# ambicuity/Distributed-LLM-Training-and-Inference-System

Measured on AMD Instinct MI355X. Metric: tokens/sec (node) GPT-7B train, higher is better.
Workload: dtype bf16; 1 GPU; model=gpt-7b, global_batch=16, seq_len=2048, parallelism=dp1, micro_batch=16, grad_accum=1, activation_checkpoint=none, layout=planner

## Files before the change

llmctl/ops/csrc/flash_attn_bwd.hip:

```cpp
#include <cstdlib>
#include <map>
#include <mutex>

#include "attn_common.h"

namespace llmctl {
using namespace attn;
namespace {

constexpr float LOG2E = 1.4426950408889634f;
constexpr int KV_KB = 128;
constexpr int KV_QT = 64;
#ifndef LLMCTL_DKV_NBUF
#define LLMCTL_DKV_NBUF 2
#endif
constexpr int KV_NBUF = LLMCTL_DKV_NBUF;
static_assert(KV_NBUF >= 2 && KV_NBUF <= 4, "dK/dV ring depth 2-4");
constexpr int DQ_QB = 128;
constexpr int DQ_KB = 64;

struct BwdArgs {
  const unsigned short *q, *k, *v, *dout;
  const float* lse;
  const float* delta;
// ... 509 lines not shown
  const unsigned short* qc = qh + (long)q_start * a.q_ss;
  const unsigned short* dc = dh + (long)q_start * a.do_ss;
  const long q_step = (long)KV_QT * a.q_ss, d_step = (long)KV_QT * a.do_ss;
  auto issue = [&](auto slot_c) __attribute__((always_inline)) {
    constexpr int SLC = decltype(slot_c)::value;
    const int nr = min(KV_QT, a.S - iq0);
    i32x4_t rq = buf_rsrc(qc, (unsigned)(((nr - 1) * a.q_ss + HD) * 2));
    i32x4_t rd = buf_rsrc(dc, (unsigned)(((nr - 1) * a.do_ss + HD) * 2));
    i32x4_t rr = (DOC && wave == 2) ? buf_rsrc(a.doc + (long)b * a.S + iq0, (unsigned)(nr * 4))
                                    : buf_rsrc(rh + iq0, (unsigned)(nr * 4));
    asm volatile("s_nop 4" : "+s"(rq), "+s"(rd), "+s"(rr));
    const unsigned slot = lds0 + (unsigned)(SLC * BUF_B);
#pragma unroll
    for (int i = 0; i < NP; ++i) {
      buf_dma16(rq, vq[i], slot + (i * 4 + wave) * 1024);
      buf_dma16(rd, vd[i], slot + TILE_B + (i * 4 + wave) * 1024);
    }
    buf_dma4(rr, rc_off, slot + 2 * TILE_B + wave * RC_B);
    iq0 += KV_QT;
    qc += q_step;
    dc += d_step;
    if (iq0 >= q_end) {
      iq0 = q_start;
      qh += a.q_sh;
      dh += a.do_sh;
      rh += a.S;
      qc = qh + (long)q_start * a.q_ss;
      dc = dh + (long)q_start * a.do_ss;
    }
  };

  const float c = a.scale_log2;
  auto apply_mask = [&](f32x16& s, int h, int q0, const int* doc_s) __attribute__((always_inline)) {
#pragma unroll
    for (int gq = 0; gq < 4; ++gq) {
      const int row0 = 32 * h + 8 * gq + 4 * hh;
      int sv[4] = {0, 0, 0, 0};
      if constexpr (DOC) {
        const int4 s4 = *reinterpret_cast<const int4*>(doc_s + row0);
        sv[0] = s4.x; sv[1] = s4.y; sv[2] = s4.z; sv[3] = s4.w;
      }
#pragma unroll
      for (int j = 0; j < 4; ++j) {
        const int qq = q0 + row0 + j;
        bool ok = qq < a.S && my_key < a.S;
        if constexpr (CAUSAL) ok = ok && my_key <= qq;
        if constexpr (DOC) ok = ok && my_key >= sv[j];
        s[4 * gq + j] = ok ? s[4 * gq + j] : -INFINITY;
      }
    }
  };

  if (ntiles > 0) issue(std::integral_constant<int, 0>{});
  bf16x8_t kf[NKS], vf[NKS];
  {
    const int kc = min(my_key, a.S - 1);
    const unsigned short* Kp = a.k + b * a.k_sb + hk * a.k_sh + (long)kc * a.k_ss + 8 * hh;
    const unsigned short* Vp = a.v + b * a.v_sb + hk * a.v_sh + (long)kc * a.v_ss + 8 * hh;
#pragma unroll
    for (int ks = 0; ks < NKS; ++ks) {
      asm volatile("global_load_dwordx4 %0, %1, off" : "=a"(kf[ks]) : "v"(Kp + 16 * ks) : "memory");
      asm volatile("global_load_dwordx4 %0, %1, off" : "=a"(vf[ks]) : "v"(Vp + 16 * ks) : "memory");
    }
  }
  vm_wait_n<0>();
  __builtin_amdgcn_s_barrier();
  stamp(2);
  if (ntiles > 1) issue(std::integral_constant<int, 1>{});
  int qi = 0;
  auto tile = [&](auto slot_c, int t) __attribute__((always_inline)) {
    constexpr int SL = decltype(slot_c)::value;
    const int q0 = q_start + qi * KV_QT;
    if (++qi == nq) qi = 0;
    const bool live = !(CAUSAL && wkey0 > q0 + KV_QT - 1);
    const unsigned char* Qs = smem + SL * BUF_B;
    const unsigned char* Ds = Qs + TILE_B;
    const float* lse_s = reinterpret_cast<const float*>(Ds + TILE_B);
    const float* del_s = lse_s + KV_QT;
    const int* doc_s = reinterpret_cast<const int*>(del_s + KV_QT);
    if (!live) return;
    f32x16 s0 = *reinterpret_cast<const f32x16*>(lse_s + 16 * hh);
    f32x16 p0 = *reinterpret_cast<const f32x16*>(del_s + 16 * hh);
    bf16x8_t qa[NKS], da[NKS];
#pragma unroll
    for (int ks = 0; ks < NKS; ++ks) {
      qa[ks] = lds_read_b128(Qs, tr_off<HD>(r, 2 * ks + hh));
      da[ks] = lds_read_b128(Ds, tr_off<HD>(r, 2 * ks + hh));
    }
    const bool need_mask = DOC || (CAUSAL && wkey0 + 31 > q0) || (q0 + KV_QT > a.S) || (wkey0 + 31 >= a.S);
#pragma unroll
    for (int ks = 0; ks < NKS; ++ks) {
      mfma_v(s0, qa[ks], kf[ks]);
      mfma_v(p0, da[ks], vf[ks]);
    }
    f32x16 s1 = *reinterpret_cast<const f32x16*>(lse_s + 32 + 16 * hh);
    f32x16 p1 = *reinterpret_cast<const f32x16*>(del_s + 32 + 16 * hh);
#pragma unroll
    for (int ks = 0; ks < NKS; ++ks) {
      qa[ks] = lds_read_b128(Qs, tr_off<HD>(32 + r, 2 * ks + hh));
      da[ks] = lds_read_b128(Ds, tr_off<HD>(32 + r, 2 * ks + hh));
    }
    if (need_mask) apply_mask(s0, 0, q0, doc_s);
    unsigned pw0[8], dw0[8];
    bf16x8_t td[2][NDB], tq[2][NDB];
#pragma unroll
    for (int ks = 0; ks < NKS; ++ks) {
      x_step(s1, p1, qa[ks], kf[ks], da[ks], vf[ks], s0[2 * ks], s0[2 * ks + 1], p0[2 * ks], p0[2 * ks + 1], c, pw0[ks],
             dw0[ks]);
      const int st = ks >> 2, d = ks & 3;
      td[st][d] = tr_frag<HD>(Ds, 16 * st, d * 32, lane);
      tq[st][d] = tr_frag<HD>(Qs, 16 * st, d * 32, lane);
    }
    if (need_mask) apply_mask(s1, 1, q0, doc_s);
    unsigned pw1[8], dw1[8];
    bf16x8_t cd[2][NDB], cq[2][NDB];
#pragma unroll
    for (int st = 0; st < 2; ++st) {
      const bf16x8_t pb = words8(pw0[4 * st], pw0[4 * st + 1], pw0[4 * st + 2], pw0[4 * st + 3]);
      const bf16x8_t sb = words8(dw0[4 * st], dw0[4 * st + 1], dw0[4 * st + 2], dw0[4 * st + 3]);
#pragma unroll
      for (int d = 0; d < NDB; ++d) {
        const int i = 4 * st + d;
        y_step(dv[d], dk[d], td[st][d], tq[st][d], pb, sb, s1[2 * i], s1[2 * i + 1], p1[2 * i], p1[2 * i + 1], c,
               pw1[i], dw1[i]);
        cd[st][d] = tr_frag<HD>(Ds, 32 + 16 * st, d * 32, lane);
        cq[st][d] = tr_frag<HD>(Qs, 32 + 16 * st, d * 32, lane);
      }
    }
#pragma unroll
    for (int st = 0; st < 2; ++st) {
      const bf16x8_t pb = words8(pw1[4 * st], pw1[4 * st + 1], pw1[4 * st + 2], pw1[4 * st + 3]);
      const bf16x8_t sb = words8(dw1[4 * st], dw1[4 * st + 1], dw1[4 * st + 2], dw1[4 * st + 3]);
#pragma unroll
      for (int d = 0; d < NDB; ++d) z_step(dv[d], dk[d], cd[st][d], cq[st][d], pb, sb);
    }
  };
  auto advance = [&](auto slot_c, int t) __attribute__((always_inline)) {
    constexpr int SL = decltype(slot_c)::value;
    asm volatile("s_waitcnt lgkmcnt(0)" ::: "memory");
    vm_wait_n<0>();
    __builtin_amdgcn_s_barrier();
    if (t + 2 < ntiles) issue(std::integral_constant<int, SL>{});
  };
  for (int t = 0; t < ntiles; t += 2) {
    tile(std::integral_constant<int, 0>{}, t);
    advance(std::integral_constant<int, 0>{}, t);
    if (t + 1 < ntiles) {
      tile(std::integral_constant<int, 1>{}, t + 1);
      advance(std::integral_constant<int, 1>{}, t + 1);
    }
  }
  stamp(3);
#pragma unroll
  for (int d = 0; d < NDB; ++d) asm volatile("s_nop 7\n\ts_nop 7" : "+a"(dk[d]), "+a"(dv[d]));
  if (my_key < a.S) {
    const long tok = (long)b * a.S + my_key;
    unsigned short* dkp = a.dk + tok * a.dk_st + (long)hk * HD;
    unsigned short* dvp = a.dv + tok * a.dv_st + (long)hk * HD;
    const float *cr = nullptr, *sr = nullptr;
    if (a.cos_t != nullptr) {
      const long p = a.rope_pos ? (long)a.rope_pos[tok] : tok % a.rope_S;
      cr = a.cos_t + p * (HD / 2);
      sr = a.sin_t + p * (HD / 2);
    }
    store_row<HD>(dkp, dk, a.scale, hh, cr, sr);
    store_row<HD>(dvp, dv, 1.f, hh, nullptr, nullptr);
  }
  if constexpr (STAMP) {
    asm volatile("s_waitcnt vmcnt(0)" ::: "memory");
    __syncthreads();
    stamp(4);
    if (tid == 0) a.stamps[blockIdx.x * 8 + 5] = (unsigned long long)ntiles;
  }
}

template <bool STAMP>
__global__ __launch_bounds__(256, 1) void fa_bwd_dkv_persist_kernel(BwdArgs a, int* __restrict__ wq) {
  constexpr int HD = 128;
  constexpr int NKS = HD / 16;
  constexpr int NDB = HD / 32;
  constexpr int ROWB = HD * 2;
  constexpr int TILE_B = KV_QT * ROWB;
  constexpr int NP = TILE_B / 1024 / 4;
  constexpr int RC_B = KV_QT * 4;
  constexpr int BUF_B = 2 * TILE_B + 4 * RC_B;
  __shared__ __attribute__((aligned(1024))) unsigned char smem[2 * BUF_B + 64];
  int* item_w = reinterpret_cast<int*>(smem + 2 * BUF_B);

  const int tid = threadIdx.x;
  const int lane = tid & 63;
  const int wave = __builtin_amdgcn_readfirstlane(tid >> 6);
  const int r = lane & 31, hh = lane >> 5;
  const int nkb = a.S / KV_KB;
  const int BH = a.B * a.Hkv;
  const bool per_xcd = BH % 8 == 0;
  const int xq = per_xcd ? (int)(blockIdx.x & 7) : 0;
  const int n_items = (per_xcd ? BH / 8 : BH) * nkb;
  const int bh_base = per_xcd ? xq * (BH / 8) : 0;
  const int group = a.Hq / a.Hkv;
  auto pop = [&]() __attribute__((always_inline)) -> int {
    const int j = __hip_atomic_fetch_add(wq + xq, 1, __ATOMIC_RELAXED, __HIP_MEMORY_SCOPE_AGENT);
    return j < n_items ? j : -1;
  };
  if (tid == 0) {
    const int i0 = pop();
    item_w[1] = i0;
    item_w[2] = i0 >= 0 ? pop() : -1;
  }
  __syncthreads();
  int cur = __builtin_amdgcn_readfirstlane(item_w[1]);
  int nxt = __builtin_amdgcn_readfirstlane(item_w[2]);
  if (cur < 0) return;

  const unsigned lds0 = lds_addr(smem);
  unsigned vq[NP], vd[NP];
#pragma unroll
  for (int i = 0; i < NP; ++i) {
    const int byte = (i * 4 + wave) * 1024 + lane * 16;
    const int row = byte / ROWB;
    const int lch = ((byte % ROWB) >> 4) ^ swz_tr<HD>(row);
    vq[i] = (unsigned)((row * a.q_ss + lch * 8) * 2);
    vd[i] = (unsigned)((row * a.do_ss + lch * 8) * 2);
  }
  const float* rc_src = a.rck_w + (wave == 1 ? a.rc_n : 0);
  const unsigned rc_off =
      (unsigned)((32 * (lane >> 5) + 8 * ((lane >> 2) & 3) + 4 * ((lane >> 4) & 1) + (lane & 3)) * 4);

  int iss = cur, iq0 = 0, iq_start = 0, ig = 0;
  const unsigned short *qh = nullptr, *dh = nullptr;
  const float* rh = nullptr;
  bool look_pending = false;
  int n_switch = 0;
  int pend0 = -1, pend1 = -1, npend = 0;
  auto iss_begin = [&](int item) __attribute__((always_inline)) {
    const int bh = bh_base + item / nkb, kb = item % nkb;
    const int bb = bh / a.Hkv, hkk = bh % a.Hkv;
    iq_start = kb * KV_KB;
    iq0 = iq_start;
    ig = 0;
    qh = a.q + bb * a.q_sb + (long)(hkk * group) * a.q_sh;
    dh = a.dout + bb * a.do_sb + (long)(hkk * group) * a.do_sh;
    rh = rc_src + ((long)bb * a.Hq + hkk * group) * a.S;
  };
  iss_begin(cur);
  auto issue = [&](auto slot_c) __attribute__((always_inline)) {
    constexpr int SLC = decltype(slot_c)::value;
    i32x4_t rq = buf_rsrc(qh + (long)iq0 * a.q_ss, (unsigned)(((KV_QT - 1) * a.q_ss + HD) * 2));
    i32x4_t rd = buf_rsrc(dh + (long)iq0 * a.do_ss, (unsigned)(((KV_QT - 1) * a.do_ss + HD) * 2));
    i32x4_t rr = buf_rsrc(rh + iq0, (unsigned)(KV_QT * 4));
    asm volatile("s_nop 4" : "+s"(rq), "+s"(rd), "+s"(rr));
    const unsigned slot = lds0 + (unsigned)(SLC * BUF_B);
#pragma unroll
    for (int i = 0; i < NP; ++i) {
      buf_dma16(rq, vq[i], slot + (i * 4 + wave) * 1024);
      buf_dma16(rd, vd[i], slot + TILE_B + (i * 4 + wave) * 1024);
    }
    buf_dma4(rr, rc_off, slot + 2 * TILE_B + wave * RC_B);
    iq0 += KV_QT;
    if (iq0 >= a.S) {
      if (++ig < group) {
        iq0 = iq_start;
        qh += a.q_sh;
        dh += a.do_sh;
        rh += a.S;
      } else {
        iss = nxt;
        if (iss >= 0) {
          iss_begin(iss);
          if (tid == 0) item_w[3 + (n_switch & 1)] = pop();
          look_pending = true;
          ++n_switch;
        }
        if (npend == 0) pend0 = iss;
        else pend1 = iss;
        ++npend;
      }
    }
  };

  bf16x8_t kf[NKS], vf[NKS];
  auto load_kv = [&](int item) __attribute__((always_inline)) {
    const int bh = bh_base + item / nkb, kb = item % nkb;
    const int bb = bh / a.Hkv, hkk = bh % a.Hkv;
    const int key = kb * KV_KB + wave * 32 + r;
    const unsigned short* Kp = a.k + bb * a.k_sb + hkk * a.k_sh + (long)key * a.k_ss + 8 * hh;
    const unsigned short* Vp = a.v + bb * a.v_sb + hkk * a.v_sh + (long)key * a.v_ss + 8 * hh;
#pragma unroll
    for (int ks = 0; ks < NKS; ++ks) {
      asm volatile("global_load_dwordx4 %0, %1, off" : "+a"(kf[ks]) : "v"(Kp + 16 * ks) : "memory");
      asm volatile("global_load_dwordx4 %0, %1, off" : "+a"(vf[ks]) : "v"(Vp + 16 * ks) : "memory");
    }
  };

  issue(std::integral_constant<int, 0>{});
  load_kv(cur);
  asm volatile("s_waitcnt vmcnt(0)"
               : "+a"(kf[0]), "+a"(kf[1]), "+a"(kf[2]), "+a"(kf[3]), "+a"(kf[4]), "+a"(kf[5]), "+a"(kf[6]),
                 "+a"(kf[7]), "+a"(vf[0]), "+a"(vf[1]), "+a"(vf[2]), "+a"(vf[3]), "+a"(vf[4]), "+a"(vf[5]),
                 "+a"(vf[6]), "+a"(vf[7])
               :
               : "memory");
  __builtin_amdgcn_s_barrier();
  issue(std::integral_constant<int, 1>{});
  f32x16 dk[NDB], dv[NDB];
#pragma unroll
  for (int d = 0; d < NDB; ++d) {
    const bf16x8_t z = {};
    asm volatile("s_nop 2\n\tv_mfma_f32_32x32x16_bf16 %0, %1, %1, 0" : "=a"(dk[d]) : "v"(z));
    asm volatile("v_mfma_f32_32x32x16_bf16 %0, %1, %1, 0" : "=a"(dv[d]) : "v"(z));
  }
  const float c = a.scale_log2;

  int n_done = 0;
  auto stamp = [&](int k) __attribute__((always_inline)) {
    if constexpr (STAMP) {
      if (tid == 0 && n_done < 64)
        a.stamps[(blockIdx.x * 64 + n_done) * 4 + k] = k == 3 ? (unsigned long long)cur : __builtin_amdgcn_s_memrealtime();
    }
  };
  for (;;) {
    stamp(0);
    stamp(3);
    const int bh = bh_base + cur / nkb, kb = cur % nkb;
    const int b = bh / a.Hkv, hk = bh % a.Hkv;
    const int k0 = kb * KV_KB;
    const int wkey0 = k0 + wave * 32;
    const int my_key = wkey0 + r;
    const int ntiles = group * ((a.S - k0) / KV_QT);
    int q0 = k0;
    auto apply_mask = [&](f32x16& s, int h) __attribute__((always_inline)) {
#pragma unroll
      for (int gq = 0; gq < 4; ++gq) {
        const int row0 = q0 + 32 * h + 8 * gq + 4 * hh;
#pragma unroll
        for (int j = 0; j < 4; ++j) s[4 * gq + j] = my_key <= row0 + j ? s[4 * gq + j] : -INFINITY;
      }
    };
    auto tile = [&](auto slot_c) __attribute__((always_inline)) {
      constexpr int SL = decltype(slot_c)::value;
      const bool live = !(wkey0 > q0 + KV_QT - 1);
      if (!live) return;
      const unsigned char* Qs = smem + SL * BUF_B;
      const unsigned char* Ds = Qs + TILE_B;
      const float* lse_s = reinterpret_cast<const float*>(Ds + TILE_B);
      const float* del_s = lse_s + KV_QT;
      const bool need_mask = wkey0 + 31 > q0;
      f32x16 s0 = *reinterpret_cast<const f32x16*>(lse_s + 16 * hh);
      f32x16 p0 = *reinterpret_cast<const f32x16*>(del_s + 16 * hh);
      bf16x8_t qa[NKS], da[NKS];
#pragma unroll
      for (int ks = 0; ks < NKS; ++ks) {
        qa[ks] = lds_read_b128(Qs, tr_off<HD>(r, 2 * ks + hh));
        da[ks] = lds_read_b128(Ds, tr_off<HD>(r, 2 * ks + hh));
      }
      f32x16 s1 = *reinterpret_cast<const f32x16*>(lse_s + 32 + 16 * hh);
      f32x16 p1 = *reinterpret_cast<const f32x16*>(del_s + 32 + 16 * hh);
      bf16x8_t qb[NKS], db[NKS];
#pragma unroll
      for (int ks = 0; ks < NKS; ++ks) {
        mfma_v(s0, qa[ks], kf[ks]);
        qb[ks] = lds_read_b128(Qs, tr_off<HD>(32 + r, 2 * ks + hh));
        mfma_v(p0, da[ks], vf[ks]);
        db[ks] = lds_read_b128(Ds, tr_off<HD>(32 + r, 2 * ks + hh));
      }
      if (need_mask) apply_mask(s0, 0);
      unsigned pw0[8], dw0[8];
      bf16x8_t td[2][NDB], tq[2][NDB];
#pragma unroll
      for (int ks = 0; ks < NKS; ++ks) {
        x_step(s1, p1, qb[ks], kf[ks], db[ks], vf[ks], s0[2 * ks], s0[2 * ks + 1], p0[2 * ks], p0[2 * ks + 1], c,
               pw0[ks], dw0[ks]);
        const int st = ks >> 2, d = ks & 3;
        td[st][d] = tr_frag<HD>(Ds, 16 * st, d * 32, lane);
        tq[st][d] = tr_frag<HD>(Qs, 16 * st, d * 32, lane);
      }
      if (need_mask) apply_mask(s1, 1);
      unsigned pw1[8], dw1[8];
      bf16x8_t cd[2][NDB], cq[2][NDB];
#pragma unroll
      for (int st = 0; st < 2; ++st) {
        const bf16x8_t pb = words8(pw0[4 * st], pw0[4 * st + 1], pw0[4 * st + 2], pw0[4 * st + 3]);
        const bf16x8_t sb = words8(dw0[4 * st], dw0[4 * st + 1], dw0[4 * st + 2], dw0[4 * st + 3]);
#pragma unroll
        for (int d = 0; d < NDB; ++d) {
          const int i = 4 * st + d;
          y_step(dv[d], dk[d], td[st][d], tq[st][d], pb, sb, s1[2 * i], s1[2 * i + 1], p1[2 * i], p1[2 * i + 1], c,
                 pw1[i], dw1[i]);
          cd[st][d] = tr_frag<HD>(Ds, 32 + 16 * st, d * 32, lane);
          cq[st][d] = tr_frag<HD>(Qs, 32 + 16 * st, d * 32, lane);
        }
      }
#pragma unroll
      for (int st = 0; st < 2; ++st) {
        const bf16x8_t pb = words8(pw1[4 * st], pw1[4 * st + 1], pw1[4 * st + 2], pw1[4 * st + 3]);
        const bf16x8_t sb = words8(dw1[4 * st], dw1[4 * st + 1], dw1[4 * st + 2], dw1[4 * st + 3]);
#pragma unroll
        for (int d = 0; d < NDB; ++d) z_step(dv[d], dk[d], cd[st][d], cq[st][d], pb, sb);
      }
    };
    auto advance = [&](auto slot_c) __attribute__((always_inline)) {
      constexpr int SL = decltype(slot_c)::value;
      asm volatile("s_waitcnt lgkmcnt(0)" ::: "memory");
      vm_wait_n<0>();
      __builtin_amdgcn_s_barrier();
      if (look_pending) {
        nxt = __builtin_amdgcn_readfirstlane(item_w[3 + ((n_switch - 1) & 1)]);
        look_pending = false;
      }
      if (iss >= 0) issue(std::integral_constant<int, SL>{});
      q0 += KV_QT;
      if (q0 >= a.S) q0 = k0;
    };
    for (int t = 0; t < ntiles; t += 2) {
      tile(std::integral_constant<int, 0>{});
      advance(std::integral_constant<int, 0>{});
      tile(std::integral_constant<int, 1>{});
      advance(std::integral_constant<int, 1>{});
    }
    stamp(1);
    {
      const long tok = (long)b * a.S + my_key;
      unsigned short* dkp = a.dk + tok * a.dk_st + (long)hk * HD;
      unsigned short* dvp = a.dv + tok * a.dv_st + (long)hk * HD;
      const bool rope = a.cos_t != nullptr;
      f32x4 cs[NDB / 2][4], sn[NDB / 2][4];
      if (rope) {
        const long p = a.rope_pos ? (long)a.rope_pos[tok] : tok % a.rope_S;
        const float* cr = a.cos_t + p * (HD / 2);
        const float* sr = a.sin_t + p * (HD / 2);
#pragma unroll
        for (int d = 0; d < NDB / 2; ++d)
#pragma unroll
          for (int g = 0; g < 4; ++g) {
            const int col = d * 32 + 8 * g + 4 * hh;
            cs[d][g] = *reinterpret_cast<const f32x4*>(cr + col);
            sn[d][g] = *reinterpret_cast<const f32x4*>(sr + col);
          }
      }
#pragma unroll
      for (int d = 0; d < NDB; ++d) asm volatile("s_nop 7\n\ts_nop 7" : "+a"(dk[d]), "+a"(dv[d]));
      auto st8 = [&](unsigned short* p, const float* x, float mul) __attribute__((always_inline)) {
        s2_t w;
        w[0] = (unsigned)f2bf(x[0] * mul) | ((unsigned)f2bf(x[1] * mul) << 16);
        w[1] = (unsigned)f2bf(x[2] * mul) | ((unsigned)f2bf(x[3] * mul) << 16);
        asm volatile("global_store_dwordx2 %0, %1, off" ::"v"(p), "v"(w) : "memory");
      };
#pragma unroll
      for (int d = 0; d < NDB / 2; ++d) {
        const f32x16 x1 = acc_copy(dk[d]), x2 = acc_copy(dk[d + NDB / 2]);
        acc_zero(dk[d]);
        acc_zero(dk[d + NDB / 2]);
#pragma unroll
        for (int g = 0; g < 4; ++g) {
          const int col = d * 32 + 8 * g + 4 * hh;
          float lo[4], hi[4];
#pragma unroll
          for (int j = 0; j < 4; ++j) {
            const float c1 = rope ? cs[d][g][j] : 1.f, s1 = rope ? sn[d][g][j] : 0.f;
            lo[j] = x1[4 * g + j] * c1 + x2[4 * g + j] * s1;
            hi[j] = x2[4 * g + j] * c1 - x1[4 * g + j] * s1;
          }
          st8(dkp + col, lo, a.scale);
          st8(dkp + col + HD / 2, hi, a.scale);
        }
      }
#pragma unroll
      for (int d = 0; d < NDB; ++d) {
        const f32x16 x = acc_copy(dv[d]);
        acc_zero(dv[d]);
#pragma unroll
        for (int g = 0; g < 4; ++g) {
          float y[4];
#pragma unroll
          for (int j = 0; j < 4; ++j) y[j] = x[4 * g + j];
          st8(dvp + d * 32 + 8 * g + 4 * hh, y, 1.f);
        }
      }
      load_kv(pend0 >= 0 ? pend0 : cur);
      asm volatile("s_waitcnt vmcnt(0)"
                   : "+a"(kf[0]), "+a"(kf[1]), "+a"(kf[2]), "+a"(kf[3]), "+a"(kf[4]), "+a"(kf[5]), "+a"(kf[6]),
                     "+a"(kf[7]), "+a"(vf[0]), "+a"(vf[1]), "+a"(vf[2]), "+a"(vf[3]), "+a"(vf[4]), "+a"(vf[5]),
                     "+a"(vf[6]), "+a"(vf[7])
                   :
                   : "memory");
    }
    stamp(2);
    ++n_done;
    if (pend0 < 0) break;
    cur = pend0;
    pend0 = pend1;
    pend1 = -1;
    --npend;
  }
}

template <int HD, bool CAUSAL, bool DOC>
__global__ __launch_bounds__(256, 2) void fa_bwd_dq_kernel(BwdArgs a) {
  constexpr int NKS = HD / 16;
  constexpr int NDB = HD / 32;
  constexpr int ROWB = HD * 2;
  constexpr int TILE = DQ_KB * ROWB;
  constexpr int PPW = TILE / 1024 / 4;
  constexpr int SLOT = 2 * TILE;
  __shared__ __attribute__((aligned(1024))) unsigned char smem[2 * SLOT];

  const int tid = threadIdx.x;
  const int lane = tid & 63;
  const int wave = __builtin_amdgcn_readfirstlane(tid >> 6);
  const int r = lane & 31, hh = lane >> 5;
  const int nqb = (a.S + DQ_QB - 1) / DQ_QB;
  const int BH = a.B * a.Hq;
  int bh, qi;
  if (BH % 8) {
    bh = blockIdx.x % BH;
    qi = blockIdx.x / BH;
  } else {
    const int x = blockIdx.x & 7, j = blockIdx.x >> 3;
    bh = x * (BH >> 3) + j / nqb;
    qi = j % nqb;
  }
  const int qblk = nqb - 1 - qi;
  const int b = bh / a.Hq, hq = bh % a.Hq;
  const int hk = hq / (a.Hq / a.Hkv);
  const int q_row0 = qblk * DQ_QB + wave * 32;
  const int my_q = q_row0 + r;
  const int qc = min(my_q, a.S - 1);

  const unsigned short* Kp = a.k + b * a.k_sb + hk * a.k_sh;
  const unsigned short* Vp = a.v + b * a.v_sb + hk * a.v_sh;

#pragma unroll
  for (int i = 0; i < 2 * SLOT / 4096; ++i)
    *reinterpret_cast<uint4*>(smem + i * 4096 + tid * 16) = make_uint4(0, 0, 0, 0);

  bf16x8_t qf[NKS], df[NKS];
  {
    const unsigned short* Qp = a.q + b * a.q_sb + hq * a.q_sh + (long)qc * a.q_ss + 8 * hh;
    const unsigned short* Dp = a.dout + b * a.do_sb + hq * a.do_sh + (long)qc * a.do_ss + 8 * hh;
#pragma unroll
    for (int ks = 0; ks < NKS; ++ks) {
      qf[ks] = __builtin_bit_cast(bf16x8_t, gload16(Qp + 16 * ks));
      df[ks] = __builtin_bit_cast(bf16x8_t, gload16(Dp + 16 * ks));
    }
  }
  const long rc = ((long)b * a.Hq + hq) * a.S + qc;
  const float nlse2 = -a.lse[rc] * LOG2E;
  float dlt;
  if (a.o != nullptr) {
    const unsigned short* Op = a.o + b * a.o_sb + hq * a.o_sh + (long)qc * a.o_ss + 8 * hh;
    float acc = 0.f;
#pragma unroll
    for (int ks = 0; ks < NKS; ++ks) {
      const bf16x8_t of = __builtin_bit_cast(bf16x8_t, gload16(Op + 16 * ks));
#pragma unroll
      for (int j = 0; j < 8; ++j) acc += (float)of[j] * (float)df[ks][j];
    }
    dlt = xor32_add(acc);
    if (hh == 0 && my_q < a.S) a.delta_w[rc] = dlt;
  } else {
    dlt = a.delta[rc];
  }
  if (hh == 0 && my_q < a.S) {
    a.rck_w[rc] = -a.lse[rc] / a.scale;
    a.rck_w[a.rc_n + rc] = -dlt;
  }
#pragma unroll
  for (int ks = 0; ks < NKS; ++ks) asm volatile("" ::"v"(qf[ks]), "v"(df[ks]));
  asm volatile("" ::"v"(nlse2), "v"(dlt));

  f32x16 dq[NDB];
#pragma unroll
  for (int d = 0; d < NDB; ++d)
#pragma unroll
    for (int i = 0; i < 16; ++i) dq[d][i] = 0.f;

  const int kv_end = CAUSAL ? min(a.S, qblk * DQ_QB + DQ_QB) : a.S;
  const int ntiles = (kv_end + DQ_KB - 1) / DQ_KB;
  int my_start = 0, w_min = 0, w_max = 0, t0 = 0;
  if constexpr (DOC) {
    const int* ds = a.doc + (long)b * a.S;
    my_start = ds[qc];
    w_min = __builtin_amdgcn_readfirstlane(ds[min(q_row0, a.S - 1)]);
    w_max = __builtin_amdgcn_readfirstlane(ds[min(q_row0 + 31, a.S - 1)]);
    t0 = __builtin_amdgcn_readfirstlane(ds[min(qblk * DQ_QB, a.S - 1)]) / DQ_KB;
  }
  const int key_hi = CAUSAL ? qc : a.S - 1;
  int klo[NDB], khi[NDB];
#pragma unroll
  for (int d = 0; d < NDB; ++d) tr_frag_offs<HD>(d * 32, lane, klo[d], khi[d]);
  int kro[NKS], vro[NKS];
#pragma unroll
  for (int ks = 0; ks < NKS; ++ks) {
    kro[ks] = tr_off<HD>(r, 2 * ks + hh);
    vro[ks] = row_off<HD>(r, 2 * ks + hh);
  }

  unsigned vk[PPW], vv[PPW];
#pragma unroll
  for (int i = 0; i < PPW; ++i) {
    const int byte = (i * 4 + wave) * 1024 + lane * 16;
    const int row = byte / ROWB, pch = (byte % ROWB) >> 4;
    vk[i] = (unsigned)((row * a.k_ss + ((pch ^ swz_tr<HD>(row)) << 3)) * 2);
    vv[i] = (unsigned)((row * a.v_ss + ((pch ^ swz_row<HD>(row)) << 3)) * 2);
  }
  const unsigned lds0 = lds_addr(smem);
  int ik0 = t0 * DQ_KB;
  const unsigned short* kc = Kp + (long)ik0 * a.k_ss;
  const unsigned short* vc = Vp + (long)ik0 * a.v_ss;
  const long k_step = (long)DQ_KB * a.k_ss, v_step = (long)DQ_KB * a.v_ss;
  auto issue = [&](auto slot_c) __attribute__((always_inline)) {
    constexpr int SLC = decltype(slot_c)::value;
    const int nk = min(DQ_KB, a.S - ik0);
    i32x4_t rk = buf_rsrc(kc, (unsigned)(((nk - 1) * a.k_ss + HD) * 2));
    i32x4_t rv = buf_rsrc(vc, (unsigned)(((nk - 1) * a.v_ss + HD) * 2));
    asm volatile("s_nop 4" : "+s"(rk), "+s"(rv));
    const unsigned slot = lds0 + (unsigned)(SLC * SLOT) + wave * 1024;
#pragma unroll
    for (int i = 0; i < PPW; ++i) {
      buf_dma16(rk, vk[i], slot + i * 4096);
      buf_dma16(rv, vv[i], slot + TILE + i * 4096);
    }
    ik0 += DQ_KB;
    kc += k_step;
    vc += v_step;
  };

  auto tile = [&](bool need_mask, const unsigned char* Ks, const unsigned char* Vs, int kv0)
                  __attribute__((always_inline)) {
#pragma unroll
    for (int kb = 0; kb < 2; ++kb) {
      f32x16 s, dp;
#pragma unroll
      for (int i = 0; i < 16; ++i) s[i] = dp[i] = 0.f;
#pragma unroll
      for (int ks = 0; ks < NKS; ++ks) {
        s = mfma32(lds_read_b128(Ks, kb * 32 * (HD * 2) + kro[ks]), qf[ks], s);
        dp = mfma32(lds_read_b128(Vs, kb * 32 * (HD * 2) + vro[ks]), df[ks], dp);
      }
      if (need_mask) {
#pragma unroll
        for (int i = 0; i < 16; ++i) {
          const int key = kv0 + kb * 32 + acc_row(i, hh);
          bool ok = key <= key_hi;
          if constexpr (DOC) ok = ok && key >= my_start;
          s[i] = ok ? s[i] : -INFINITY;
        }
      }
      float dsv[16];
#pragma unroll
      for (int i = 0; i < 16; ++i) dsv[i] = fast_exp2(__builtin_fmaf(s[i], a.scale_log2, nlse2)) * (dp[i] - dlt);
#pragma unroll
      for (int st = 0; st < 2; ++st) {
        const bf16x8_t sbf = to_bf16x8(dsv + 8 * st);
#pragma unroll
        for (int d = 0; d < NDB; ++d) dq[d] = mfma32(tr_frag_at<HD>(Ks, kb * 32 + 16 * st, klo[d], khi[d]), sbf, dq[d]);
      }
    }
  };

  __syncthreads();
  auto step = [&](auto slot_c, int t) __attribute__((always_inline)) {
    constexpr int SL = decltype(slot_c)::value;
    vm_wait_n<0>();
    __builtin_amdgcn_s_barrier();
    if (t + 1 < ntiles) issue(std::integral_constant<int, 1 - SL>{});
    const int kv0 = t * DQ_KB;
    bool live = true;
    if constexpr (CAUSAL) live = kv0 <= q_row0 + 31;
    if constexpr (DOC) live = live && kv0 + DQ_KB > w_min;
    if (live) {
      const bool need_mask =
          (CAUSAL && kv0 + DQ_KB - 1 > q_row0) || (kv0 + DQ_KB > a.S) || (DOC && kv0 < w_max);
      tile(need_mask, smem + SL * SLOT, smem + SL * SLOT + TILE, kv0);
    }
  };
  if (t0 < ntiles) issue(std::integral_constant<int, 0>{});
  for (int t = t0; t < ntiles; t += 2) {
    step(std::integral_constant<int, 0>{}, t);
    if (t + 1 < ntiles) step(std::integral_constant<int, 1>{}, t + 1);
  }
  if (my_q < a.S) {
    const long tok = (long)b * a.S + my_q;
    const float *cr = nullptr, *sr = nullptr;
    if (a.cos_t != nullptr) {
      const long p = a.rope_pos ? (long)a.rope_pos[tok] : tok % a.rope_S;
      cr = a.cos_t + p * (HD / 2);
      sr = a.sin_t + p * (HD / 2);
    }
    store_row<HD>(a.dq + tok * a.dq_st + (long)hq * HD, dq, a.scale, hh, cr, sr);
  }
}

int dkv_mode() {
  const int64_t m = knob("dkv", 2);
  return (m >= 0 && m <= 2) ? (int)m : 2;
}

int* dkv_queue(hipStream_t s) {
  static std::mutex mu;
  static std::map<std::pair<int, hipStream_t>, int*> bufs;
  int dev = 0;
  LLMCTL_HIP_CHECK(hipGetDevice(&dev));
  std::lock_guard<std::mutex> lk(mu);
  int*& q = bufs[{dev, s}];
  if (q == nullptr) LLMCTL_HIP_CHECK(hipMalloc(&q, 64 * sizeof(int)));
  return q;
}

template <int HD, bool CAUSAL, bool DOC>
void launch_bwd(const BwdArgs& a, hipStream_t s, bool do_dq, bool do_dkv, int dkv_impl) {
  if (do_dq) {
    const int nqb = (a.S + DQ_QB - 1) / DQ_QB;
    hipLaunchKernelGGL((fa_bwd_dq_kernel<HD, CAUSAL, DOC>), dim3((unsigned)(a.B * a.Hq * nqb)), dim3(256), 0, s, a);
  }
  if (do_dkv) {
    const int nkb = (a.S + KV_KB - 1) / KV_KB;
    const dim3 grid((unsigned)(a.B * a.Hkv * nkb));
    if constexpr (HD == 128 && CAUSAL) {
      if (dkv_impl == 2 && a.stamps != nullptr) {
        hipLaunchKernelGGL((fa_bwd_dkv_pipe_kernel<HD, CAUSAL, DOC, true>), grid, dim3(256), 0, s, a);
        return;
      }
      if constexpr (!DOC) {
        if (a.S % KV_KB == 0 && (dkv_impl == 3 || dkv_impl == 4 || (dkv_impl < 0 && dkv_mode() == 2))) {
          int* wq = dkv_queue(s);
          LLMCTL_HIP_CHECK(hipMemsetAsync(wq, 0, 8 * sizeof(int), s));
          int nwg = std::min<long>((long)num_cus(), (long)a.B * a.Hkv * nkb);
          const int min_wg = ((long)a.B * a.Hkv) % 8 == 0 ? 8 : 1;
          if (const int64_t e = knob("dkv_nwg", 0); e > 0) nwg = std::max<int>(min_wg, std::min<int>(nwg, (int)e));
          nwg = std::max(nwg, min_wg);
          if (a.stamps != nullptr)
            hipLaunchKernelGGL(fa_bwd_dkv_persist_kernel<true>, dim3((unsigned)nwg), dim3(256), 0, s, a, wq);
          else
            hipLaunchKernelGGL(fa_bwd_dkv_persist_kernel<false>, dim3((unsigned)nwg), dim3(256), 0, s, a, wq);
          return;
        }
      }
      if (dkv_impl == 1 || dkv_impl == 3 || (dkv_impl < 0 && dkv_mode() >= 1)) {
        hipLaunchKernelGGL((fa_bwd_dkv_pipe_kernel<HD, CAUSAL, DOC>), grid, dim3(256), 0, s, a);
        return;
      }
    }
    hipLaunchKernelGGL((fa_bwd_dkv_kernel<HD, CAUSAL, DOC>), grid, dim3(256), 0, s, a);
  }
}

void dispatch_bwd(const BwdArgs& a, int D, bool causal, bool doc, hipStream_t s, bool do_dq = true,
                  bool do_dkv = true, int dkv_impl = -1) {
  if (doc) {
    if (D == 128) launch_bwd<128, true, true>(a, s, do_dq, do_dkv, dkv_impl);
    else launch_bwd<64, true, true>(a, s, do_dq, do_dkv, dkv_impl);
  } else if (D == 128) {
    if (causal) launch_bwd<128, true, false>(a, s, do_dq, do_dkv, dkv_impl);
    else launch_bwd<128, false, false>(a, s, do_dq, do_dkv, dkv_impl);
  } else {
    if (causal) launch_bwd<64, true, false>(a, s, do_dq, do_dkv, dkv_impl);
    else launch_bwd<64, false, false>(a, s, do_dq, do_dkv, dkv_impl);
  }
}

BwdArgs make_args(const at::Tensor& dout, const at::Tensor& q, const at::Tensor& k, const at::Tensor& v,
                  const at::Tensor& lse, const at::Tensor& delta, at::Tensor& dq, at::Tensor& dk, at::Tensor& dv,
                  double scale) {
  return BwdArgs{bf_ptr(q), bf_ptr(k), bf_ptr(v), bf_ptr(dout), lse.data_ptr<float>(), delta.data_ptr<float>(),
                 bf_mut(dq), bf_mut(dk), bf_mut(dv), (int)q.size(0), (int)q.size(1), (int)q.size(2),
                 (int)k.size(2), q.stride(0), q.stride(1), q.stride(2), k.stride(0), k.stride(1), k.stride(2),
                 v.stride(0), v.stride(1), v.stride(2), dout.stride(0), dout.stride(1), dout.stride(2),
                 (float)scale, (float)(scale * 1.4426950408889634), nullptr,
                 (long)dq.size(2) * dq.size(3), (long)dk.size(2) * dk.size(3), (long)dv.size(2) * dv.size(3),
                 nullptr, nullptr, nullptr, 0, nullptr, 0, 0, 0, nullptr, nullptr, 0};
}

at::Tensor row_consts(BwdArgs& a, const at::Tensor& lse) {
  auto rck = at::empty({2 * lse.numel()}, lse.options());
  a.rck_w = rck.data_ptr<float>();
  a.rc_n = lse.numel();
  return rck;
}

}

std::tuple<at::Tensor, at::Tensor, at::Tensor> flash_attn_bwd(const at::Tensor& dout, const at::Tensor& q,
                                                              const at::Tensor& k, const at::Tensor& v,
                                                              const at::Tensor& o, const at::Tensor& lse,
                                                              double scale, bool causal,
                                                              const c10::optional<at::Tensor>& doc_start) {
  LLMCTL_CHECK(q.dim() == 4 && k.dim() == 4 && v.dim() == 4 && o.dim() == 4 && dout.dim() == 4,
               "flash_attn_bwd: [B,S,H,D] tensors");
  const int B = q.size(0), S = q.size(1), Hq = q.size(2), D = q.size(3);
  const int Hkv = k.size(2);
  LLMCTL_CHECK(D == 64 || D == 128, "head_dim must be 64 or 128");
  LLMCTL_CHECK(Hkv > 0 && Hq % Hkv == 0, "Hq must be a multiple of Hkv");
  LLMCTL_CHECK(dout.sizes() == q.sizes() && o.sizes() == q.sizes() && k.sizes() == v.sizes() && k.size(0) == B &&
                   k.size(1) == S && k.size(3) == D,
               "shape mismatch");
  LLMCTL_CHECK(lse.scalar_type() == at::kFloat && lse.is_contiguous() && lse.numel() == (long)B * Hq * S,
// ... 126 lines not shown
```

Baseline: 30680 tokens/s.

## Software-pipeline dK/dV bwd tiles: prefetch next tile's Q/dO fragments and next K/V

Restructures the dK/dV backward inner loop so the barrier and next-slot issue happen mid-tile, and the next tile's lse/delta and Q/dO row-0 fragments are read from LDS during the current tile's final z_step MFMAs. The next work item's K/V loads are issued during the last tile instead of after the dK/dV epilogue, with a partial vmcnt wait covering the outstanding stores. Transpose fragment offsets are precomputed once. It aims to hide LDS and global latency behind MFMA work, at the cost of higher register pressure and fragile vmcnt accounting.

```diff
diff --git a/llmctl/ops/csrc/flash_attn_bwd.hip b/llmctl/ops/csrc/flash_attn_bwd.hip
--- a/llmctl/ops/csrc/flash_attn_bwd.hip
+++ b/llmctl/ops/csrc/flash_attn_bwd.hip
@@ -835,6 +835,24 @@
                : "memory");
   __builtin_amdgcn_s_barrier();
   issue(std::integral_constant<int, 1>{});
+  int tlo[NDB], thi[NDB];
+#pragma unroll
+  for (int d = 0; d < NDB; ++d) tr_frag_offs<HD>(d * 32, lane, tlo[d], thi[d]);
+  f32x16 s0, p0;
+  bf16x8_t qa[NKS], da[NKS];
+  auto r0_consts = [&](auto slot_c) __attribute__((always_inline)) {
+    const float* lse_s = reinterpret_cast<const float*>(smem + decltype(slot_c)::value * BUF_B + 2 * TILE_B);
+    s0 = *reinterpret_cast<const f32x16*>(lse_s + 16 * hh);
+    p0 = *reinterpret_cast<const f32x16*>(lse_s + KV_QT + 16 * hh);
+  };
+  auto r0_frag = [&](auto slot_c, int ks) __attribute__((always_inline)) {
+    const unsigned char* Qs = smem + decltype(slot_c)::value * BUF_B;
+    qa[ks] = lds_read_b128(Qs, tr_off<HD>(r, 2 * ks + hh));
+    da[ks] = lds_read_b128(Qs + TILE_B, tr_off<HD>(r, 2 * ks + hh));
+  };
+  r0_consts(std::integral_constant<int, 0>{});
+#pragma unroll
+  for (int ks = 0; ks < NKS; ++ks) r0_frag(std::integral_constant<int, 0>{}, ks);
   f32x16 dk[NDB], dv[NDB];
 #pragma unroll
   for (int d = 0; d < NDB; ++d) {
@@ -869,86 +887,98 @@
         for (int j = 0; j < 4; ++j) s[4 * gq + j] = my_key <= row0 + j ? s[4 * gq + j] : -INFINITY;
       }
     };
-    auto tile = [&](auto slot_c) __attribute__((always_inline)) {
+    auto tile = [&](auto slot_c, auto last_c) __attribute__((always_inline)) {
       constexpr int SL = decltype(slot_c)::value;
-      const bool live = !(wkey0 > q0 + KV_QT - 1);
-      if (!live) return;
+      const bool last = last_c;
+      using other = std::integral_constant<int, SL ^ 1>;
       const unsigned char* Qs = smem + SL * BUF_B;
       const unsigned char* Ds = Qs + TILE_B;
       const float* lse_s = reinterpret_cast<const float*>(Ds + TILE_B);
       const float* del_s = lse_s + KV_QT;
-      const bool need_mask = wkey0 + 31 > q0;
-      f32x16 s0 = *reinterpret_cast<const f32x16*>(lse_s + 16 * hh);
-      f32x16 p0 = *reinterpret_cast<const f32x16*>(del_s + 16 * hh);
-      bf16x8_t qa[NKS], da[NKS];
-#pragma unroll
-      for (int ks = 0; ks < NKS; ++ks) {
-        qa[ks] = lds_read_b128(Qs, tr_off<HD>(r, 2 * ks + hh));
-        da[ks] = lds_read_b128(Ds, tr_off<HD>(r, 2 * ks + hh));
-      }
-      f32x16 s1 = *reinterpret_cast<const f32x16*>(lse_s + 32 + 16 * hh);
-      f32x16 p1 = *reinterpret_cast<const f32x16*>(del_s + 32 + 16 * hh);
-      bf16x8_t qb[NKS], db[NKS];
-#pragma unroll
-      for (int ks = 0; ks < NKS; ++ks) {
-        mfma_v(s0, qa[ks], kf[ks]);
-        qb[ks] = lds_read_b128(Qs, tr_off<HD>(32 + r, 2 * ks + hh));
-        mfma_v(p0, da[ks], vf[ks]);
-        db[ks] = lds_read_b128(Ds, tr_off<HD>(32 + r, 2 * ks + hh));
-      }
-      if (need_mask) apply_mask(s0, 0);
-      unsigned pw0[8], dw0[8];
-      bf16x8_t td[2][NDB], tq[2][NDB];
-#pragma unroll
-      for (int ks = 0; ks < NKS; ++ks) {
-        x_step(s1, p1, qb[ks], kf[ks], db[ks], vf[ks], s0[2 * ks], s0[2 * ks + 1], p0[2 * ks], p0[2 * ks + 1], c,
-               pw0[ks], dw0[ks]);
-        const int st = ks >> 2, d = ks & 3;
-        td[st][d] = tr_frag<HD>(Ds, 16 * st, d * 32, lane);
-        tq[st][d] = tr_frag<HD>(Qs, 16 * st, d * 32, lane);
-      }
-      if (need_mask) apply_mask(s1, 1);
+      auto boundary = [&]() __attribute__((always_inline)) {
+        asm volatile("s_waitcnt lgkmcnt(0)" ::: "memory");
+        if (last) vm_wait_n<2 * NKS>();
+        else vm_wait_n<0>();
+        __builtin_amdgcn_s_barrier();
+        if (look_pending) {
+          nxt = __builtin_amdgcn_readfirstlane(item_w[3 + ((n_switch - 1) & 1)]);
+          look_pending = false;
+        }
+        if (iss >= 0) issue(std::integral_constant<int, SL>{});
+      };
+      const bool live = !(wkey0 > q0 + KV_QT - 1);
       unsigned pw1[8], dw1[8];
       bf16x8_t cd[2][NDB], cq[2][NDB];
-#pragma unroll
-      for (int st = 0; st < 2; ++st) {
-        const bf16x8_t pb = words8(pw0[4 * st], pw0[4 * st + 1], pw0[4 * st + 2], pw0[4 * st + 3]);
-        const bf16x8_t sb = words8(dw0[4 * st], dw0[4 * st + 1], dw0[4 * st + 2], dw0[4 * st + 3]);
-#pragma unroll
-        for (int d = 0; d < NDB; ++d) {
-          const int i = 4 * st + d;
-          y_step(dv[d], dk[d], td[st][d], tq[st][d], pb, sb, s1[2 * i], s1[2 * i + 1], p1[2 * i], p1[2 * i + 1], c,
-                 pw1[i], dw1[i]);
-          cd[st][d] = tr_frag<HD>(Ds, 32 + 16 * st, d * 32, lane);
-          cq[st][d] = tr_frag<HD>(Qs, 32 + 16 * st, d * 32, lane);
-        }
-      }
+      if (live) {
+        const bool need_mask = wkey0 + 31 > q0;
+        f32x16 s1, p1;
+        bf16x8_t qb[NKS], db[NKS];
+#pragma unroll
+        for (int ks = 0; ks < NKS; ++ks) {
+          mfma_v(s0, qa[ks], kf[ks]);
+          qb[ks] = lds_read_b128(Qs, tr_off<HD>(32 + r, 2 * ks + hh));
+          mfma_v(p0, da[ks], vf[ks]);
+          db[ks] = lds_read_b128(Ds, tr_off<HD>(32 + r, 2 * ks + hh));
+          if (ks == 1) s1 = *reinterpret_cast<const f32x16*>(lse_s + 32 + 16 * hh);
+          if (ks == 3) p1 = *reinterpret_cast<const f32x16*>(del_s + 32 + 16 * hh);
+        }
+        if (need_mask) apply_mask(s0, 0);
+        unsigned pw0[8], dw0[8];
+        bf16x8_t td[2][NDB], tq[2][NDB];
+#pragma unroll
+        for (int ks = 0; ks < NKS; ++ks) {
+          x_step(s1, p1, qb[ks], kf[ks], db[ks], vf[ks], s0[2 * ks], s0[2 * ks + 1], p0[2 * ks], p0[2 * ks + 1], c,
+                 pw0[ks], dw0[ks]);
+          const int st = ks >> 2, d = ks & 3;
+          td[st][d] = tr_frag_at<HD>(Ds, 16 * st, tlo[d], thi[d]);
+          tq[st][d] = tr_frag_at<HD>(Qs, 16 * st, tlo[d], thi[d]);
+        }
+        if (last) load_kv(pend0 >= 0 ? pend0 : cur);
+        if (need_mask) apply_mask(s1, 1);
+#pragma unroll
+        for (int st = 0; st < 2; ++st) {
+          const bf16x8_t pb = words8(pw0[4 * st], pw0[4 * st + 1], pw0[4 * st + 2], pw0[4 * st + 3]);
+          const bf16x8_t sb = words8(dw0[4 * st], dw0[4 * st + 1], dw0[4 * st + 2], dw0[4 * st + 3]);
+#pragma unroll
+          for (int d = 0; d < NDB; ++d) {
+            const int i = 4 * st + d;
+            y_step(dv[d], dk[d], td[st][d], tq[st][d], pb, sb, s1[2 * i], s1[2 * i + 1], p1[2 * i], p1[2 * i + 1], c,
+                   pw1[i], dw1[i]);
+            cd[st][d] = tr_frag_at<HD>(Ds, 32 + 16 * st, tlo[d], thi[d]);
+            cq[st][d] = tr_frag_at<HD>(Qs, 32 + 16 * st, tlo[d], thi[d]);
+          }
+        }
+      } else {
+#pragma unroll
+        for (int i = 0; i < 8; ++i) {
+          pw1[i] = dw1[i] = 0u;
+          cd[i >> 2][i & 3] = cq[i >> 2][i & 3] = bf16x8_t{};
+        }
+      }
+      boundary();
+      r0_consts(other{});
 #pragma unroll
       for (int st = 0; st < 2; ++st) {
         const bf16x8_t pb = words8(pw1[4 * st], pw1[4 * st + 1], pw1[4 * st + 2], pw1[4 * st + 3]);
         const bf16x8_t sb = words8(dw1[4 * st], dw1[4 * st + 1], dw1[4 * st + 2], dw1[4 * st + 3]);
 #pragma unroll
-        for (int d = 0; d < NDB; ++d) z_step(dv[d], dk[d], cd[st][d], cq[st][d], pb, sb);
+        for (int d = 0; d < NDB; ++d) {
+          z_step(dv[d], dk[d], cd[st][d], cq[st][d], pb, sb);
+          r0_frag(other{}, 4 * st + d);
+        }
       }
     };
-    auto advance = [&](auto slot_c) __attribute__((always_inline)) {
-      constexpr int SL = decltype(slot_c)::value;
-      asm volatile("s_waitcnt lgkmcnt(0)" ::: "memory");
-      vm_wait_n<0>();
-      __builtin_amdgcn_s_barrier();
-      if (look_pending) {
-        nxt = __builtin_amdgcn_readfirstlane(item_w[3 + ((n_switch - 1) & 1)]);
-        look_pending = false;
-      }
-      if (iss >= 0) issue(std::integral_constant<int, SL>{});
+    auto next_rows = [&]() __attribute__((always_inline)) {
       q0 += KV_QT;
       if (q0 >= a.S) q0 = k0;
     };
+    using slot0 = std::integral_constant<int, 0>;
+    using slot1 = std::integral_constant<int, 1>;
     for (int t = 0; t < ntiles; t += 2) {
-      tile(std::integral_constant<int, 0>{});
-      advance(std::integral_constant<int, 0>{});
-      tile(std::integral_constant<int, 1>{});
-      advance(std::integral_constant<int, 1>{});
+      tile(slot0{}, std::false_type{});
+      next_rows();
+      tile(slot1{}, t + 2 >= ntiles);
+      next_rows();
     }
     stamp(1);
     {
@@ -1009,8 +1039,11 @@
           st8(dvp + d * 32 + 8 * g + 4 * hh, y, 1.f);
         }
       }
-      load_kv(pend0 >= 0 ? pend0 : cur);
-      asm volatile("s_waitcnt vmcnt(0)"
+      r0_consts(slot0{});
+#pragma unroll
+      for (int ks = 0; ks < NKS; ++ks) r0_frag(slot0{}, ks);
+      static_assert(NDB * 8 == 32, "the wait's immediate counts the dK / dV stores");
+      asm volatile("s_waitcnt vmcnt(32)"
                    : "+a"(kf[0]), "+a"(kf[1]), "+a"(kf[2]), "+a"(kf[3]), "+a"(kf[4]), "+a"(kf[5]), "+a"(kf[6]),
                      "+a"(kf[7]), "+a"(vf[0]), "+a"(vf[1]), "+a"(vf[2]), "+a"(vf[3]), "+a"(vf[4]), "+a"(vf[5]),
                      "+a"(vf[6]), "+a"(vf[7])
@@ -1025,6 +1058,7 @@
     pend1 = -1;
     --npend;
   }
+  asm volatile("s_waitcnt vmcnt(0)" ::: "memory");
 }
 
 template <int HD, bool CAUSAL, bool DOC>
```

New measurement: 30840 tokens/s, median of 6. About the same (+0.5%).
